# magicat777/Audio-Analyzer-OMEGA

Hardware: AMD Instinct MI355X
Metric: audio frames/sec (multi-res FFT + LUFS + TruePeak) at 1/2/4/8 MI355X (higher is better)
Workload: dtype f32; 1 GPU; cfg2: 256 stereo frames x 16384 samples per GPU; MRFFT 16k/8k/4k/1k + combine(512) + K-weighted LUFS + 4x true peak + meter aggregates; channel_frames_per_gpu=512, frame_samples=16384, target_bins=512, parallelism=frames sharded over 1 GPU(s)

## Files before the change

audio-analyzer-omega_amd/csrc/regfft.hpp:

```cpp
#pragma once
#include "fft.hpp"

namespace omega {

__device__ constexpr float kCos128[16] = {
    1.000000000e+00f, 9.987954562e-01f, 9.951847267e-01f, 9.891765100e-01f, 9.807852804e-01f,
    9.700312532e-01f, 9.569403357e-01f, 9.415440652e-01f, 9.238795325e-01f, 9.039892931e-01f,
    8.819212643e-01f, 8.577286100e-01f, 8.314696123e-01f, 8.032075315e-01f, 7.730104534e-01f,
    7.409511254e-01f};
__device__ constexpr float kSin128[16] = {
    0.000000000e+00f, 4.906767433e-02f, 9.801714033e-02f, 1.467304745e-01f, 1.950903220e-01f,
    2.429801799e-01f, 2.902846773e-01f, 3.368898534e-01f, 3.826834324e-01f, 4.275550934e-01f,
    4.713967368e-01f, 5.141027442e-01f, 5.555702330e-01f, 5.956993045e-01f, 6.343932842e-01f,
    6.715589548e-01f};

__device__ __forceinline__ void wave_lds_sync() {
  asm volatile("s_waitcnt lgkmcnt(0)" ::: "memory");
  __builtin_amdgcn_wave_barrier();
}

__device__ __forceinline__ float lane_xor1(float v) {
  return __int_as_float(__builtin_amdgcn_mov_dpp(__float_as_int(v), 0xB1, 0xF, 0xF, true));
}

__device__ __forceinline__ void lane_pair_fmac(float2 (&v)[16], float s) {
  asm volatile(
      "s_nop 1\n"
      "v_fmac_f32_dpp %0, %0, %32 quad_perm:[1,0,3,2] row_mask:0xf bank_mask:0xf\n"
      "v_fmac_f32_dpp %1, %1, %32 quad_perm:[1,0,3,2] row_mask:0xf bank_mask:0xf\n"
      "v_fmac_f32_dpp %2, %2, %32 quad_perm:[1,0,3,2] row_mask:0xf bank_mask:0xf\n"
      "v_fmac_f32_dpp %3, %3, %32 quad_perm:[1,0,3,2] row_mask:0xf bank_mask:0xf\n"
      "v_fmac_f32_dpp %4, %4, %32 quad_perm:[1,0,3,2] row_mask:0xf bank_mask:0xf\n"
      "v_fmac_f32_dpp %5, %5, %32 quad_perm:[1,0,3,2] row_mask:0xf bank_mask:0xf\n"
      "v_fmac_f32_dpp %6, %6, %32 quad_perm:[1,0,3,2] row_mask:0xf bank_mask:0xf\n"
      "v_fmac_f32_dpp %7, %7, %32 quad_perm:[1,0,3,2] row_mask:0xf bank_mask:0xf\n"
      "v_fmac_f32_dpp %8, %8, %32 quad_perm:[1,0,3,2] row_mask:0xf bank_mask:0xf\n"
      "v_fmac_f32_dpp %9, %9, %32 quad_perm:[1,0,3,2] row_mask:0xf bank_mask:0xf\n"
      "v_fmac_f32_dpp %10, %10, %32 quad_perm:[1,0,3,2] row_mask:0xf bank_mask:0xf\n"
      "v_fmac_f32_dpp %11, %11, %32 quad_perm:[1,0,3,2] row_mask:0xf bank_mask:0xf\n"
      "v_fmac_f32_dpp %12, %12, %32 quad_perm:[1,0,3,2] row_mask:0xf bank_mask:0xf\n"
      "v_fmac_f32_dpp %13, %13, %32 quad_perm:[1,0,3,2] row_mask:0xf bank_mask:0xf\n"
      "v_fmac_f32_dpp %14, %14, %32 quad_perm:[1,0,3,2] row_mask:0xf bank_mask:0xf\n"
      "v_fmac_f32_dpp %15, %15, %32 quad_perm:[1,0,3,2] row_mask:0xf bank_mask:0xf\n"
      "v_fmac_f32_dpp %16, %16, %32 quad_perm:[1,0,3,2] row_mask:0xf bank_mask:0xf\n"
      "v_fmac_f32_dpp %17, %17, %32 quad_perm:[1,0,3,2] row_mask:0xf bank_mask:0xf\n"
      "v_fmac_f32_dpp %18, %18, %32 quad_perm:[1,0,3,2] row_mask:0xf bank_mask:0xf\n"
      "v_fmac_f32_dpp %19, %19, %32 quad_perm:[1,0,3,2] row_mask:0xf bank_mask:0xf\n"
      "v_fmac_f32_dpp %20, %20, %32 quad_perm:[1,0,3,2] row_mask:0xf bank_mask:0xf\n"
      "v_fmac_f32_dpp %21, %21, %32 quad_perm:[1,0,3,2] row_mask:0xf bank_mask:0xf\n"
      "v_fmac_f32_dpp %22, %22, %32 quad_perm:[1,0,3,2] row_mask:0xf bank_mask:0xf\n"
      "v_fmac_f32_dpp %23, %23, %32 quad_perm:[1,0,3,2] row_mask:0xf bank_mask:0xf\n"
      "v_fmac_f32_dpp %24, %24, %32 quad_perm:[1,0,3,2] row_mask:0xf bank_mask:0xf\n"
      "v_fmac_f32_dpp %25, %25, %32 quad_perm:[1,0,3,2] row_mask:0xf bank_mask:0xf\n"
      "v_fmac_f32_dpp %26, %26, %32 quad_perm:[1,0,3,2] row_mask:0xf bank_mask:0xf\n"
      "v_fmac_f32_dpp %27, %27, %32 quad_perm:[1,0,3,2] row_mask:0xf bank_mask:0xf\n"
      "v_fmac_f32_dpp %28, %28, %32 quad_perm:[1,0,3,2] row_mask:0xf bank_mask:0xf\n"
      "v_fmac_f32_dpp %29, %29, %32 quad_perm:[1,0,3,2] row_mask:0xf bank_mask:0xf\n"
      "v_fmac_f32_dpp %30, %30, %32 quad_perm:[1,0,3,2] row_mask:0xf bank_mask:0xf\n"
      "v_fmac_f32_dpp %31, %31, %32 quad_perm:[1,0,3,2] row_mask:0xf bank_mask:0xf\n"
      : "+v"(v[0].x), "+v"(v[0].y),
        "+v"(v[1].x), "+v"(v[1].y),
        "+v"(v[2].x), "+v"(v[2].y),
        "+v"(v[3].x), "+v"(v[3].y),
        "+v"(v[4].x), "+v"(v[4].y),
        "+v"(v[5].x), "+v"(v[5].y),
        "+v"(v[6].x), "+v"(v[6].y),
        "+v"(v[7].x), "+v"(v[7].y),
        "+v"(v[8].x), "+v"(v[8].y),
        "+v"(v[9].x), "+v"(v[9].y),
        "+v"(v[10].x), "+v"(v[10].y),
        "+v"(v[11].x), "+v"(v[11].y),
        "+v"(v[12].x), "+v"(v[12].y),
        "+v"(v[13].x), "+v"(v[13].y),
        "+v"(v[14].x), "+v"(v[14].y),
        "+v"(v[15].x), "+v"(v[15].y)
      : "v"(s));
}

struct WinGen {
  float c0, c1, c2;
  float4 base;
  float4 step[8];
  __device__ __forceinline__ WinGen(const float4* __restrict__ g, int t) {
    const float4 c = g[0];
    c0 = c.x;
    c1 = c.y;
    c2 = c.z;
#pragma unroll
    for (int i = 0; i < 8; ++i) step[i] = g[1 + i];
    base = g[9 + t];
  }
  template <int Q, bool C2 = true>
  __device__ __forceinline__ float2 at() const {
    const float4 s4 = step[Q / 2];
    const float cs = (Q & 1) ? s4.z : s4.x, sn = (Q & 1) ? s4.w : s4.y;
    const float C0 = fmaf(base.x, cs, -base.y * sn), C1 = fmaf(base.z, cs, -base.w * sn);
    if constexpr (C2) return make_float2(fmaf(C0, fmaf(c2, C0, c1), c0), fmaf(C1, fmaf(c2, C1, c1), c0));
    else return make_float2(fmaf(C0, c1, c0), fmaf(C1, c1, c0));
  }
};

template <int K>
struct RegFFT {
  static_assert(K == 8192 || K == 4096, "register FFT plans: K = 4096, 8192");
  static constexpr int NTH = K / 16;
  static constexpr int L = K / 256;
  static constexpr int P1 = L == 32 ? 544 : 272;
  static constexpr int P2R = L == 32 ? 544 : 272;
  static constexpr int P2C = L == 32 ? 34 : 17;
  static_assert(P1 == P2R && 16 * P2R <= (K == 8192 ? 8712 : 4352), "exchange rows shared by both exchanges");
  static constexpr int kSlots = K == 8192 ? 8712 : 4352;
  static constexpr int kT2 = 15 * L;

  static __device__ __forceinline__ int a3(int n) {
    if constexpr (K == 8192) return n + (n >> 4) + ((n >> 12) << 3);
    else return n ^ ((n >> 4) & 15);
  }
  static __device__ __forceinline__ int s3(int t) {
    if constexpr (K == 8192) return t + (t >> 4);
    else return t ^ ((t >> 4) & 15);
  }
  static constexpr int o3(int r) { return K == 8192 ? 544 * r + 8 * (r >> 3) : 256 * r; }
  static __device__ __forceinline__ int s3m(int t) { return s3(NTH - t); }
  static __device__ __forceinline__ int out_index(int s, int m) {
    if constexpr (L == 32) return (s >> 5) + 16 * ((s >> 1) & 15) + 256 * (m + 16 * (s & 1));
    else return (s >> 4) + 16 * (s & 15) + 256 * m;
  }
  static __device__ __forceinline__ int s3o(int s) {
    if constexpr (L == 32) return (s >> 5) + 17 * ((s >> 1) & 15) + 4360 * (s & 1);
    else return ((s >> 4) ^ (s & 15)) + 16 * (s & 15);
  }
  static constexpr int o3o(int m) { return L == 32 ? 272 * m : 256 * m; }

  static __device__ __forceinline__ void twiddle(float2 (&v)[16], float2 w) {
    float2 wk = w;
    static_for<1, 16>([&](auto k) {
      v[k] = cmul(v[k], wk);
      if constexpr (k + 1 < 16) wk = cmul(wk, w);
    });
  }

  static __device__ __forceinline__ void dft16(float2 (&v)[16]) { dft16_fma(v); }

  static __device__ __forceinline__ void fill_t2(float2* t2, const float2* __restrict__ twK, int tid) {
    for (int i = tid; i < kT2; i += NTH) {
      const int k2 = i / L + 1, u = i % L;
      t2[i] = twK[(16 * u * k2) & (K - 1)];
    }
  }
  static __device__ __forceinline__ void twiddle_t2(float2 (&v)[16], const float2* t2u) {
    static_for<1, 16>([&](auto k2) { v[k2] = cmul(v[k2], t2u[(k2 - 1) * L]); });
  }

  template <bool SYNC = false, bool LT2 = false>
  static __device__ __forceinline__ void run(float2 (&v)[16], float2* buf, int t, float2 w1, float2 w2,
                                             const float2* t2 = nullptr) {
    run2<SYNC, LT2>(v, buf, t, t, w1, w2, t2);
  }
  template <bool SYNC = false, bool LT2 = false>
  static __device__ __forceinline__ void run2(float2 (&v)[16], float2* buf, int t1, int t, float2 w1, float2 w2,
                                              const float2* t2 = nullptr) {
    dft16(v);
    twiddle(v, w1);
    if constexpr (SYNC) __syncthreads();
    {
      float2* b = buf + t1;
      static_for<0, 16>([&](auto k1) { b[P1 * k1] = v[k1]; });
    }
    __syncthreads();
    {
      const int u = t % L, k1 = t / L;
      const float2* b = buf + P1 * k1 + u;
      static_for<0, 16>([&](auto r) { v[r] = b[L * r]; });
      dft16(v);
      if constexpr (LT2)
        twiddle_t2(v, t2 + u);
      else
        twiddle(v, w2);
      float2* bw = buf + P2R * k1 + u;
      static_for<0, 16>([&](auto k2) { bw[P2C * k2] = v[k2]; });
    }
    wave_lds_sync();
    if constexpr (L == 16) {
      const int k2 = t & 15, k1 = t >> 4;
      const float2* b = buf + P2R * k1 + P2C * k2;
      static_for<0, 16>([&](auto r) { v[r] = b[r]; });
      dft16(v);
    } else {
      const int q = t & 1, k2 = (t >> 1) & 15, k1 = t >> 5;
      const float2* b = buf + P2R * k1 + P2C * k2 + q;
      static_for<0, 16>([&](auto r) { v[r] = b[2 * r]; });
      dft16(v);
      static_for<0, 16>([&](auto m) {
        const float2 tw = twc<m + 16, 32>(v[m]);
        v[m] = make_float2(q ? tw.x : v[m].x, q ? tw.y : v[m].y);
      });
      lane_pair_fmac(v, q ? 1.f : -1.f);
    }
  }

  template <bool SYNC = false, bool LT2 = false>
  static __device__ __forceinline__ void run_low(float2 (&v)[16], float2* buf, int t, float2 w1, float2 w2,
                                                 const float2* t2 = nullptr) {
    static_assert(L == 32, "the two-band pass 3 is the K = 8192 plan");
    dft16(v);
    twiddle(v, w1);
    if constexpr (SYNC) __syncthreads();
    {
      float2* b = buf + t;
      static_for<0, 16>([&](auto k1) { b[P1 * k1] = v[k1]; });
    }
    __syncthreads();
    {
      const int u = t % L, k1 = t / L;
      const float2* b = buf + P1 * k1 + u;
      static_for<0, 16>([&](auto r) { v[r] = b[L * r]; });
      dft16(v);
      if constexpr (LT2)
        twiddle_t2(v, t2 + u);
      else
        twiddle(v, w2);
      float2* bw = buf + P2R * k1 + u;
      static_for<0, 16>([&](auto k2) { bw[P2C * k2] = v[k2]; });
    }
    wave_lds_sync();
    const int q = t & 1, k2 = (t >> 1) & 15, k1 = t >> 5;
    {
      const float2* b = buf + P2R * k1 + P2C * k2 + q;
      static_for<0, 16>([&](auto r) { v[r] = b[2 * r]; });
    }
    float2 f0 = v[0], f15 = v[0];
    static_for<1, 16>([&](auto r) {
      f0 = cadd(f0, v[r]);
      f15 = cadd(f15, twc<15 * r, 16>(v[r]));
    });
    const float2 g = twc<15, 32>(f15);
    const float2 send = q ? f0 : f15;
    const float2 recv = make_float2(lane_xor1(send.x), lane_xor1(send.y));
    const float2 out = q ? csub(recv, g) : cadd(f0, recv);
    __syncthreads();
    buf[s3o(t) + (q ? o3o(15) : 0)] = out;
    __syncthreads();
  }

  template <bool LT2 = false>
  static __device__ __forceinline__ void run_half(float2 (&v)[16], float* bf, int t, float2 w1, float2 w2,
                                                  const float2* t2 = nullptr) {
    static_assert(L == 16, "the half-buffer plan is K = 4096");
    dft16(v);
    twiddle(v, w1);
    const int u = t % L, k1 = t / L;
    {
      float* b = bf + t;
      static_for<0, 16>([&](auto j) { b[P1 * j] = v[j].x; });
    }
    __syncthreads();
    {
      const float* b = bf + P1 * k1 + u;
      static_for<0, 16>([&](auto r) { v[r].x = b[L * r]; });
    }
    __syncthreads();
    {
      float* b = bf + t;
      static_for<0, 16>([&](auto j) { b[P1 * j] = v[j].y; });
    }
    __syncthreads();
    {
      const float* b = bf + P1 * k1 + u;
      static_for<0, 16>([&](auto r) { v[r].y = b[L * r]; });
    }
    dft16(v);
    if constexpr (LT2)
      twiddle_t2(v, t2 + u);
    else
      twiddle(v, w2);
    {
      float* bw = bf + P2R * k1 + u;
      static_for<0, 16>([&](auto j) { bw[P2C * j] = v[j].x; });
    }
    wave_lds_sync();
    const int k2 = t & 15, k1b = t >> 4;
    const float* br = bf + P2R * k1b + P2C * k2;
    static_for<0, 16>([&](auto r) { v[r].x = br[r]; });
    {
      float* bw = bf + P2R * k1 + u;
      static_for<0, 16>([&](auto j) { bw[P2C * j] = v[j].y; });
    }
    wave_lds_sync();
    static_for<0, 16>([&](auto r) { v[r].y = br[r]; });
    dft16(v);
  }
  template <bool IM>
  static __device__ __forceinline__ void store_spectrum_half(const float2 (&v)[16], float* bf, int t) {
    float* b = bf + s3o(t);
    static_for<0, 16>([&](auto m) { b[o3o(m)] = IM ? v[m].y : v[m].x; });
  }

  static __device__ __forceinline__ void store_spectrum(const float2 (&v)[16], float2* buf, int t) {
    float2* b = buf + s3o(t);
    static_for<0, 16>([&](auto m) { b[o3o(m)] = v[m]; });
  }
};

}
```

audio-analyzer-omega_amd/csrc/rfkern.hip:

```cpp
#include <cstdlib>

#include "stamps.hpp"

namespace omega {
OMEGA_STAMPS_DECL
OMEGA_WGTRACE_DECL
OMEGA_MARKS_DECL
}

#include "kw.hpp"
#include "meter_query.hpp"
#include "regfft.hpp"
#include "spectral.hpp"

namespace omega {

template <int K>
constexpr size_t t2_offset() { return (RegFFT<K>::kSlots + 8) * sizeof(float2) + 64; }
template <int K>
constexpr size_t lds_bytes() { return t2_offset<K>() + RegFFT<K>::kT2 * sizeof(float2); }
template <int K>
__device__ __forceinline__ float2* t2_table(char* smem) { return reinterpret_cast<float2*>(smem + t2_offset<K>()); }

template <int NTH>
__device__ __forceinline__ int tp_column(int tid) {
  const int w = tid >> 6, l = tid & 63;
  if (l < 32) return 32 * w + l;
  const int a = 32 * w + (63 - l);
  return a == 0 ? NTH / 2 : NTH - a;
}

__device__ __forceinline__ void max3_abs16(float& acc, const float2 (&a)[16]) {
  asm(
      "v_max3_f32 %0, |%1|, |%2|, %0\n"
      "v_max3_f32 %0, |%3|, |%4|, %0\n"
      "v_max3_f32 %0, |%5|, |%6|, %0\n"
      "v_max3_f32 %0, |%7|, |%8|, %0\n"
      "v_max3_f32 %0, |%9|, |%10|, %0\n"
      "v_max3_f32 %0, |%11|, |%12|, %0\n"
      "v_max3_f32 %0, |%13|, |%14|, %0\n"
      "v_max3_f32 %0, |%15|, |%16|, %0\n"
      "v_max3_f32 %0, |%17|, |%18|, %0\n"
      "v_max3_f32 %0, |%19|, |%20|, %0\n"
      "v_max3_f32 %0, |%21|, |%22|, %0\n"
      "v_max3_f32 %0, |%23|, |%24|, %0\n"
      "v_max3_f32 %0, |%25|, |%26|, %0\n"
      "v_max3_f32 %0, |%27|, |%28|, %0\n"
      "v_max3_f32 %0, |%29|, |%30|, %0\n"
      "v_max3_f32 %0, |%31|, |%32|, %0\n"
      : "+v"(acc)
      : "v"(a[0].x), "v"(a[0].y),
        "v"(a[1].x), "v"(a[1].y),
        "v"(a[2].x), "v"(a[2].y),
        "v"(a[3].x), "v"(a[3].y),
        "v"(a[4].x), "v"(a[4].y),
        "v"(a[5].x), "v"(a[5].y),
        "v"(a[6].x), "v"(a[6].y),
        "v"(a[7].x), "v"(a[7].y),
        "v"(a[8].x), "v"(a[8].y),
        "v"(a[9].x), "v"(a[9].y),
        "v"(a[10].x), "v"(a[10].y),
        "v"(a[11].x), "v"(a[11].y),
        "v"(a[12].x), "v"(a[12].y),
        "v"(a[13].x), "v"(a[13].y),
        "v"(a[14].x), "v"(a[14].y),
        "v"(a[15].x), "v"(a[15].y));
}

template <int K>
__device__ __forceinline__ void truepeak_rf_body(const SpectralParams& p, int64_t cf, int tid, char* smem) {
  using FFT = RegFFT<K>;
  constexpr int NTH = FFT::NTH, M = 2 * K;
  const int t = tp_column<NTH>(tid);
  float2* buf = reinterpret_cast<float2*>(smem);
  float* red = reinterpret_cast<float*>(smem + (FFT::kSlots + 8) * sizeof(float2));
  const int64_t f = cf / p.C, c = cf % p.C;
  const float2* x2 = reinterpret_cast<const float2*>(p.x + f * p.frame_stride + c * p.chan_stride);
  const float2* __restrict__ twK = p.tw[ilog2(K)];
  const float2* __restrict__ twM = p.tw[ilog2(M)];
  float2 v[16];
  float mx = 0.f;
  OMEGA_STAMP(0);
  const float2 w1 = twK[t], w2 = twK[16 * (tid % FFT::L)];
  const float2 wm = twM[t];
  const float2 rho = p.rot[t];
  float2* t2 = t2_table<K>(smem);
  FFT::fill_t2(t2, twK, tid);
  asm volatile("" ::: "memory");
  static_for<0, 16>([&](auto r) {
    v[r] = x2[t + NTH * r];
    mx = fmaxf(mx, fmaxf(fabsf(v[r].x), fabsf(v[r].y)));
  });
  asm volatile("" : "+v"(mx));
  OMEGA_STAMP(1);
  FFT::template run2<false, true>(v, buf, t, tid, w1, w2, t2);
  OMEGA_STAMP(2);
  __syncthreads();
  FFT::store_spectrum(v, buf, tid);
  __syncthreads();
  OMEGA_STAMP(3);
  float xn = 0.f;
  {
    const float2* bo = buf + FFT::s3(t);
    const float2* bm = buf + FFT::s3m(t);
    static_for<0, 16>([&](auto r) {
      const float2 a = bo[FFT::o3(r)];
      float2 b = bm[FFT::o3(15 - r)];
      if constexpr (K == 8192 && r == 8) {
        if (t == 0) b = a;
      }
      float2 xk, xkk;
      untangle(a, b, twc<r, 32>(wm), xk, xkk);
      if constexpr (r == 0) {
        if (t == 0) {
          xn = a.x - a.y;
          xk = make_float2(a.x + a.y, 0.f);
        }
      }
      v[r] = xk;
    });
  }
  float2 y[16];
  static_for<0, 16>([&](auto r) { y[r] = v[r]; });
  const float2 hz = make_float2(wm.y, wm.x);
  float fmx = 0.f;
  const int lane = tid & 63;
  const int mir_addr = 4 * ((t == 0 || t == NTH / 2) ? lane : lane ^ 63);
  OMEGA_STAMP(4);
#pragma unroll 1
  for (int P = 1; P <= 3; ++P) {
    int tl = t, tidl = tid;
    float2 w1l = w1, w2l = w2, rhol = rho, hzl = hz;
    asm volatile("" : "+v"(tl), "+v"(tidl), "+v"(w1l.x), "+v"(w1l.y), "+v"(w2l.x), "+v"(w2l.y));
    asm volatile("" : "+v"(rhol.x), "+v"(rhol.y), "+v"(hzl.x), "+v"(hzl.y));
    static_for<0, 16>([&](auto r) {
      const float2 rk = cmul(rhol, make_float2(kCos128[r], kSin128[r]));
      y[r] = cmul(y[r], rk);
    });
    if (!((p.tp_phases >> P) & 1)) continue;
    OMEGA_STAMP(1 + 4 * P);
    const float cp = P == 1 ? 7.071067812e-01f : (P == 2 ? 0.f : -7.071067812e-01f);
    OMEGA_STAMP(2 + 4 * P);
    static_for<0, 16>([&](auto r) {
      const float2 m = y[15 - r];
      float2 yp = make_float2(__int_as_float(__builtin_amdgcn_ds_bpermute(mir_addr, __float_as_int(m.x))),
                              -__int_as_float(__builtin_amdgcn_ds_bpermute(mir_addr, __float_as_int(m.y))));
      if constexpr (r == 0) {
        if (tl == 0) yp = make_float2(xn * cp, 0.f);
      } else {
        if (tl == 0) yp = cconj(y[16 - r]);
      }
      const float2 g = twc<-r, 32>(hzl);
      const float2 S = cadd(y[r], yp), D = csub(y[r], yp);
      v[r] = make_float2(fmaf(g.x, D.x, fmaf(-g.y, D.y, S.x)), fmaf(-g.x, D.y, fmaf(-g.y, D.x, -S.y)));
    });
    OMEGA_STAMP(3 + 4 * P);
    FFT::template run2<true, true>(v, buf, tl, tidl, w1l, w2l, t2);
    max3_abs16(fmx, v);
#if defined(OMEGA_EXP_STALL)
    asm volatile("s_sleep %0" ::"i"(OMEGA_EXP_STALL));
#endif
#if defined(OMEGA_EXP_VALU)
    {
      float d0 = fmx, d1 = mx, d2 = fmx + 1.f, d3 = mx + 1.f;
      asm volatile(".rept %4\n v_fma_f32 %0, %0, %5, %6\n v_fma_f32 %1, %1, %5, %6\n"
                   " v_fma_f32 %2, %2, %5, %6\n v_fma_f32 %3, %3, %5, %6\n .endr"
                   : "+v"(d0), "+v"(d1), "+v"(d2), "+v"(d3)
                   : "i"(OMEGA_EXP_VALU), "v"(0.5f), "v"(0.25f));
    }
#endif
    OMEGA_STAMP(4 + 4 * P);
  }
  const float peak = block_max<NTH>(fmaxf(mx, fmx * (0.5f / K)), red, tid);
  if (tid == 0) {
    const float db = peak < 1e-10f ? -100.0f : 20.0f * log10f(peak);
    if (p.tp_done) {
      __hip_atomic_store(reinterpret_cast<unsigned*>(p.tp_out + cf), __float_as_uint(db), __ATOMIC_RELAXED,
                         __HIP_MEMORY_SCOPE_AGENT);
      asm volatile("s_waitcnt vmcnt(0)" ::: "memory");
      __hip_atomic_fetch_add(p.tp_done, 1u, __ATOMIC_RELAXED, __HIP_MEMORY_SCOPE_AGENT);
    } else {
      p.tp_out[cf] = db;
    }
    if (p.tp_copy) p.tp_copy[cf] = db;
  }
}

template <int K>
__global__ __launch_bounds__(K / 16, 4) void truepeak_rf_kernel(SpectralParams p) {
  extern __shared__ __attribute__((aligned(16))) char smem[];
  OMEGA_WG_BEGIN();
  truepeak_rf_body<K>(p, blockIdx.x, threadIdx.x, smem);
  OMEGA_WG_END(1);
}

template <int K>
__device__ __forceinline__ void mrfft_rf_body(const SpectralParams& p, int r, int64_t cf, int t, char* smem) {
  using FFT = RegFFT<K>;
  constexpr int NTH = FFT::NTH, M = 2 * K;
  float2* buf = reinterpret_cast<float2*>(smem);
  const int64_t f = cf / p.C, c = cf % p.C;
  const ResParam& rp = p.res[r];
  const float2* x2 = reinterpret_cast<const float2*>(p.x + f * p.frame_stride + c * p.chan_stride + rp.offset);
  const float2* __restrict__ twK = p.tw[ilog2(K)];
  const float2* __restrict__ twM = p.tw[ilog2(M)];
  float2 v[16];
  const float2 w1 = twK[t], w2b = twK[16 * (t % FFT::L)];
  const float2 wm = twM[t];
  float2* t2 = t2_table<K>(smem);
  FFT::fill_t2(t2, twK, t);
  asm volatile("" ::: "memory");
  const float2* w2 = reinterpret_cast<const float2*>(rp.win);
  static_for<0, 16>([&](auto q) {
    const float2 a = x2[t + NTH * q], w = w2[t + NTH * q];
    v[q] = make_float2(a.x * w.x, a.y * w.y);
  });
  const int e0 = rp.ent_begin + t;
  CombEnt ent{};
  if (p.comb_out && e0 < rp.ent_end) ent = p.ent[e0];
  bool low = false;
  if constexpr (K == 8192) low = !rp.mag_out && rp.low_band;
  if (low) {
    if constexpr (K == 8192) FFT::template run_low<false, true>(v, buf, t, w1, w2b, t2);
  } else {
    FFT::template run<false, true>(v, buf, t, w1, w2b, t2);
    __syncthreads();
    FFT::store_spectrum(v, buf, t);
    __syncthreads();
  }
  if (!rp.mag_out) {
    if (!p.comb_out) return;
    auto mag_at = [&](int j) -> float {
      const float2 a = buf[FFT::a3(j == K ? 0 : j)];
      if (j == 0) return fabsf(a.x + a.y);
      if (j == K) return fabsf(a.x - a.y);
      if (j == K / 2) return cabs(a);
      const float2 b = buf[FFT::a3(K - j)];
      float2 xk, xkk;
      untangle(a, b, twM[j], xk, xkk);
      return cabs(xk);
    };
    float* o = p.comb_out + cf * p.T;
    auto apply = [&](const CombEnt& en) {
      const int tt = en.tm & 0xFFFFFF, op = en.tm >> 24;
      if (op == 2) {
        o[tt] = 0.f;
        return;
      }
      const float val = fmaf(en.c1, mag_at(en.j + 1), en.c0 * mag_at(en.j));
      if (op == 0)
        o[tt] = val;
      else
        o[tt] += val;
    };
    if (e0 < rp.ent_end) apply(ent);
    for (int e = e0 + NTH; e < rp.ent_end; e += NTH) apply(p.ent[e]);
    return;
  }
  float mg[16];
  float mnyq = 0.f;
  {
    const float2* bo = buf + FFT::s3(t);
    const float2* bm = buf + FFT::s3m(t);
    static_for<0, 16>([&](auto q) {
      const float2 a = bo[FFT::o3(q)];
      float2 b = bm[FFT::o3(15 - q)];
      if constexpr (K == 8192 && q == 8) {
        if (t == 0) b = a;
      }
      float2 xk, xkk;
      untangle(a, b, twc<q, 32>(wm), xk, xkk);
      mg[q] = cabs(xk);
      if constexpr (q == 0) {
        if (t == 0) {
          mg[0] = fabsf(a.x + a.y);
          mnyq = fabsf(a.x - a.y);
        }
      }
    });
  }
  if (rp.mag_out) {
    float* o = rp.mag_out + cf * (K + 1);
    const float* __restrict__ wgt = rp.wgt;
    static_for<0, 16>([&](auto q) { o[t + NTH * q] = mg[q] * wgt[t + NTH * q]; });
    if (t == 0) o[K] = mnyq * wgt[K];
  }
  if (!p.comb_out) return;
  float* mag = reinterpret_cast<float*>(smem);
  __syncthreads();
  static_for<0, 16>([&](auto q) { mag[t + NTH * q] = mg[q]; });
  if (t == 0) mag[K] = mnyq;
  __syncthreads();
  float* o = p.comb_out + cf * p.T;
  auto apply = [&](const CombEnt& en) {
    const int tt = en.tm & 0xFFFFFF, op = en.tm >> 24;
    const float val = fmaf(en.c1, mag[en.j + 1], en.c0 * mag[en.j]);
    if (op == 0)
      o[tt] = val;
    else if (op == 1)
      o[tt] += val;
    else
      o[tt] = 0.f;
  };
  if (e0 < rp.ent_end) apply(ent);
  for (int e = e0 + NTH; e < rp.ent_end; e += NTH) apply(p.ent[e]);
}

template <int K>
__global__ __launch_bounds__(K / 16, 4) void mrfft_rf_kernel(SpectralParams p, int r) {
  extern __shared__ __attribute__((aligned(16))) char smem[];
  OMEGA_WG_BEGIN();
  mrfft_rf_body<K>(p, r, blockIdx.x, threadIdx.x, smem);
  OMEGA_WG_END(2);
}

OMEGA_STAMPS_GETTER(omega_debug_rf_stamps)
OMEGA_WGTRACE_GETTER(omega_debug_wgtrace)
OMEGA_MARKS_GETTER(omega_debug_marks_batch)

hipError_t launch_mrfft_rf(int n, const SpectralParams& p, int r, hipStream_t s) {
  const dim3 grid((unsigned)p.n_cf);
  if (n == 16384) {
    hipLaunchKernelGGL(mrfft_rf_kernel<8192>, grid, dim3(512), lds_bytes<8192>(), s, p, r);
  } else if (n == 8192) {
    hipLaunchKernelGGL(mrfft_rf_kernel<4096>, grid, dim3(256), lds_bytes<4096>(), s, p, r);
  } else {
    return hipErrorInvalidValue;
  }
  return hipGetLastError();
}

constexpr int kSpecRfThreads = 256;
#ifndef OMEGA_SPEC_WGS
#define OMEGA_SPEC_WGS 5
#endif
constexpr int kSpecRfWgs = OMEGA_SPEC_WGS;
constexpr int kSpecRfPeakWords = 12;
template <int K>
struct SpecRfLds {
  static constexpr size_t kT2Off = RegFFT<K>::kSlots * sizeof(float);
  static constexpr size_t kXform = kT2Off + RegFFT<K>::kT2 * sizeof(float2);
  static constexpr size_t kPartOff = ((K + 1) * sizeof(float) + 15) / 16 * 16;
  static constexpr size_t kClsOff = kPartOff + 240 * 5 * sizeof(float);
  static constexpr size_t kRedOff = kClsOff + 12 * 5 * sizeof(double);
  static constexpr size_t kFlagOff = (kRedOff + (RegFFT<K>::NTH / 64) * sizeof(float) + 15) / 16 * 16;
  static constexpr int kFlagWords = 2 * 64 * kSpecRfPeakWords / 4;
  static constexpr size_t kPost = kFlagOff + kFlagWords * sizeof(unsigned);
  static constexpr size_t kBytes = kXform > kPost ? kXform : kPost;
  static_assert((kBytes + 1279) / 1280 * 1280 * kSpecRfWgs <= 160 * 1024, "LDS of kSpecRfWgs workgroups per CU");
};


template <int K>
__device__ __forceinline__ void spectra_rf_body(const SpectraParams& p) {
  using FFT = RegFFT<K>;
  constexpr int NTH = FFT::NTH;
  static_assert(NTH == kSpecRfThreads, "one 256-thread workgroup per frame");
  extern __shared__ __attribute__((aligned(16))) char smem[];
  using Lds = SpecRfLds<K>;
  float* bf = reinterpret_cast<float*>(smem);
  float* magc = reinterpret_cast<float*>(smem);
  constexpr int kFlagWords = Lds::kFlagWords;
  float* part = reinterpret_cast<float*>(smem + Lds::kPartOff);
  double(*cls)[5] = reinterpret_cast<double(*)[5]>(smem + Lds::kClsOff);
  float* redf = reinterpret_cast<float*>(smem + Lds::kRedOff);
  unsigned* sflag = reinterpret_cast<unsigned*>(smem + Lds::kFlagOff);
  const int t = threadIdx.x;
  const int64_t fr = blockIdx.x;
  const float2* x2 = reinterpret_cast<const float2*>(p.x + fr * p.stride);
  float2 v[16];
  const float2* __restrict__ twK = p.tw[ilog2(K)];
  const float2 w1 = twK[t], w2b = twK[16 * (t % FFT::L)];
  const float2 wm = p.tw[ilog2(2 * K)][t];
  float2* t2 = reinterpret_cast<float2*>(smem + Lds::kT2Off);
  FFT::fill_t2(t2, twK, t);
  constexpr int kGrp = 20;
  int bs[2] = {0, 0}, be[2] = {0, 0};
  float bsc[2] = {1.f, 1.f};
  static_for<0, 2>([&](auto j) {
    const int i = t + NTH * j;
    if (p.bands_out && i < p.n_valid) {
      bs[j] = p.starts[i];
      be[j] = p.ends[i];
      if (p.scale) bsc[j] = p.scale[i];
    }
  });
  int cj0 = 0, cj1 = 0;
  if (p.chroma_out && t < 12 * kGrp) {
    cj0 = p.cgoff[t / kGrp];
    cj1 = p.cgoff[t / kGrp + 1];
  }
  const WinGen wg(p.wgen, t);
  asm volatile("" ::: "memory");
  OMEGA_STAMP_RT(30);
  OMEGA_STAMP(0);
  if (wg.c2 == 0.f) {
    static_for<0, 16>([&](auto r) {
      const float2 a = x2[t + NTH * r], w = wg.template at<r, false>();
      v[r] = make_float2(a.x * w.x, a.y * w.y);
    });
  } else {
    static_for<0, 16>([&](auto r) {
      const float2 a = x2[t + NTH * r], w = wg.template at<r>();
      v[r] = make_float2(a.x * w.x, a.y * w.y);
    });
  }
  OMEGA_STAMP(1);
  FFT::template run_half<true>(v, bf, t, w1, w2b, t2);
  OMEGA_STAMP(2);
  constexpr int kRecPre = 2, kRecReg = 8;
  float3 ra[kRecReg];
  const float3* __restrict__ crec = reinterpret_cast<const float3*>(p.crec);
  int cjf = cj0 + t % kGrp;
  static_for<0, kRecPre>([&](auto i) {
    const int j = cjf + kGrp * i;
    if (j < cj1) {
      ra[i] = crec[j];
    }
  });
  asm volatile("" ::: "memory");
  float ax[8], bx[8], ay[8], by[8];
  float hx = 0.f, hy = 0.f;
  {
    const float* bo = bf + FFT::s3(t);
    const float* bm = bf + FFT::s3m(t);
    __syncthreads();
    FFT::template store_spectrum_half<false>(v, bf, t);
    __syncthreads();
    static_for<0, 8>([&](auto q) {
      ax[q] = bo[FFT::o3(q)];
      bx[q] = bm[FFT::o3(15 - q)];
    });
    if (t == 0) hx = bo[FFT::o3(8)];
    __syncthreads();
    FFT::template store_spectrum_half<true>(v, bf, t);
    __syncthreads();
    static_for<0, 8>([&](auto q) {
      ay[q] = bo[FFT::o3(q)];
      by[q] = bm[FFT::o3(15 - q)];
    });
    if (t == 0) hy = bo[FFT::o3(8)];
  }
  OMEGA_STAMP(3);
  float mg[8], mgm[8];
  float mx = 0.f, mhalf = 0.f;
  {
    static_for<0, 8>([&](auto q) {
      const float2 a = make_float2(ax[q], ay[q]);
      const float2 b = make_float2(bx[q], by[q]);
      float2 xk, xkk;
      untangle(a, b, twc<q, 32>(wm), xk, xkk);
      mg[q] = cabs(xk);
      mgm[q] = cabs(xkk);
      if constexpr (q == 0) {
        if (t == 0) {
          mg[0] = fabsf(a.x + a.y);
          mgm[0] = fabsf(a.x - a.y);
        }
      }
      mx = fmaxf(mx, fmaxf(mg[q], mgm[q]));
    });
    if (t == 0) {
      mhalf = cabs(make_float2(hx, hy));
      mx = fmaxf(mx, mhalf);
    }
  }
  mx = wave_max(mx);
  __syncthreads();
  static_for<0, 8>([&](auto q) {
    magc[t + NTH * q] = mg[q];
    magc[K - t - NTH * q] = mgm[q];
  });
  if (t == 0) magc[K / 2] = mhalf;
  if ((t & 63) == 0) redf[t >> 6] = mx;
  for (int i = t; i < kFlagWords; i += NTH) sflag[i] = 0u;
  OMEGA_STAMP(4);
  __syncthreads();
  float thr = redf[0];
#pragma unroll
  for (int w = 1; w < NTH / 64; ++w) thr = fmaxf(thr, redf[w]);
  thr *= 0.1f;
  if (p.chroma_out && t < 12 * kGrp) {
    static_for<0, kRecReg>([&](auto i) {
      const int j = cjf + kGrp * i;
      if (i >= kRecPre && j < cj1) {
        ra[i] = crec[j];
      }
    });
  }
  OMEGA_STAMP(5);
  if (p.mag_out) {
    float* o = p.mag_out + fr * (K + 1);
    static_for<0, 8>([&](auto q) {
      o[t + NTH * q] = mg[q];
      o[K - t - NTH * q] = mgm[q];
    });
    if (t == 0) o[K / 2] = mhalf;
  }
  if (p.bands_out) {
    float* o = p.bands_out + fr * p.n_out;
    auto band = [&](int i, int s, int e, float scale) {
      float val = 0.f;
      if (i < p.n_valid && s < K + 1 && e <= K + 1) {
        float m0 = magc[s], m1 = m0, m2 = m0, m3 = m0;
        int k = s + 1;
        for (; k + 3 < e; k += 4) {
          m0 = fmaxf(m0, magc[k]);
          m1 = fmaxf(m1, magc[k + 1]);
          m2 = fmaxf(m2, magc[k + 2]);
          m3 = fmaxf(m3, magc[k + 3]);
        }
        for (; k < e; ++k) m0 = fmaxf(m0, magc[k]);
        val = fmaxf(fmaxf(m0, m1), fmaxf(m2, m3)) * scale;
      }
      o[i] = val;
    };
    static_for<0, 2>([&](auto j) {
      const int i = t + NTH * j;
      if (i < p.n_out) {
        band(i, bs[j], be[j], bsc[j]);
      }
    });
    for (int i = t + 2 * NTH; i < p.n_out; i += NTH) {
      float val = 0.f;
      if (i < p.n_valid) {
        const int s = p.starts[i], e = p.ends[i];
        if (s < K + 1 && e <= K + 1) {
          float m0 = magc[s], m1 = m0, m2 = m0, m3 = m0;
          int k = s + 1;
          for (; k + 3 < e; k += 4) {
            m0 = fmaxf(m0, magc[k]);
            m1 = fmaxf(m1, magc[k + 1]);
            m2 = fmaxf(m2, magc[k + 2]);
            m3 = fmaxf(m3, magc[k + 3]);
          }
          for (; k < e; ++k) m0 = fmaxf(m0, magc[k]);
          val = fmaxf(fmaxf(m0, m1), fmaxf(m2, m3)) * (p.scale ? p.scale[i] : 1.f);
        }
      }
      o[i] = val;
    }
  }
  OMEGA_STAMP(6);
  if (!p.chroma_out) return;
  {
    const int lane = t & 63;
    static_for<0, kSpecRfPeakWords / (NTH / 64)>([&](auto q) {
      const int k = t + NTH * q;
      const float val = mg[q];
      float lo = wave_shift1<true>(val), hi = wave_shift1<false>(val);
      if (lane == 0) lo = k >= 1 ? magc[k - 1] : 0.f;
      if (lane == 63) hi = magc[k + 1];
      if (k >= 1 && k <= K - 1 && val > lo && val > hi && val > thr) {
        static_for<2, 6>([&](auto h) {
          const int kh = k * h;
          if (kh >= p.c_lo && kh < p.c_hi) atomicOr(&sflag[kh >> 2], 1u << (8 * (kh & 3) + h));
        });
      }
    });
  }
  __syncthreads();
  OMEGA_STAMP(7);
  auto suppressed = [&](int k) {
    const unsigned f = (sflag[k >> 2] >> (8 * (k & 3))) & 0xFFu;
    float m = magc[k];
    m = (f & 32u) ? m * (1.0f / 5) : m;
    m = (f & 16u) ? m * (1.0f / 4) : m;
    m = (f & 8u) ? m * (1.0f / 3) : m;
    m = (f & 4u) ? m * (1.0f / 2) : m;
    return m;
  };
  OMEGA_STAMP(8);
  if (t < 12 * kGrp) {
    float acc[5] = {0.f, 0.f, 0.f, 0.f, 0.f};
    const int j1 = cj1;
    auto acc_rec = [&](const float3 r) {
      const float ed = suppressed(__float_as_int(r.z));
      const float a = r.x, g = r.y, gi = __builtin_amdgcn_rcpf(g);
      const float ag = a * g, agi = a * gi;
      acc[0] = fmaf(ed, agi * (gi * 3.3546262790251185e-4f), acc[0]);
      acc[1] = fmaf(ed, agi * 1.3533528323661270e-1f, acc[1]);
      acc[2] = fmaf(ed, a, acc[2]);
      acc[3] = fmaf(ed, ag * 1.3533528323661270e-1f, acc[3]);
      acc[4] = fmaf(ed, ag * (g * 3.3546262790251185e-4f), acc[4]);
    };
    static_for<0, kRecReg>([&](auto i) {
      if (cjf + kGrp * i < j1) acc_rec(ra[i]);
    });
    for (int j = cjf + kGrp * kRecReg; j < j1; j += kGrp) acc_rec(crec[j]);
#pragma unroll
    for (int o = 0; o < 5; ++o) part[t * 5 + o] = acc[o];
  }
  OMEGA_STAMP(9);
  __syncthreads();
  OMEGA_STAMP(10);
  if (t < 60 * 4) {
    const int pr = t >> 2, k = t & 3, g = pr / 5, o = pr % 5;
    const float* pp = part + (g * kGrp + 5 * k) * 5 + o;
    double sgo = (double)pp[0];
#pragma unroll
    for (int r = 1; r < 5; ++r) sgo += (double)pp[5 * r];
    sgo += __shfl_xor(sgo, 1, 64);
    sgo += __shfl_xor(sgo, 2, 64);
    if (k == 0) cls[(g + o + 10) % 12][o] = sgo;
  }
  __syncthreads();
  if (t < 64) {
    const int c = t % 12;
    const double ch = cls[c][0] + cls[c][1] + cls[c][2] + cls[c][3] + cls[c][4];
    const int cm = (c + 11) % 12, cp = (c + 1) % 12;
    const double chm = cls[cm][0] + cls[cm][1] + cls[cm][2] + cls[cm][3] + cls[cm][4];
    const double chp = cls[cp][0] + cls[cp][1] + cls[cp][2] + cls[cp][3] + cls[cp][4];
    const double sm = 0.25 * chm + 0.5 * ch + 0.25 * chp;
    double tot = t < 12 ? sm : 0.0;
    tot += __shfl_xor(tot, 8, 64);
    tot += __shfl_xor(tot, 4, 64);
    tot += __shfl_xor(tot, 2, 64);
    tot += __shfl_xor(tot, 1, 64);
    if (t < 12) p.chroma_out[fr * 12 + c] = tot > 0 ? sm / tot : sm;
  }
  OMEGA_STAMP(11);
  OMEGA_STAMP_RT(31);
}

template <int K>
__global__ __launch_bounds__(kSpecRfThreads, kSpecRfWgs) void spectra_rf_kernel(SpectraParams p) {
  OMEGA_WG_BEGIN();
  spectra_rf_body<K>(p);
  OMEGA_WG_END(20);
}

hipError_t launch_spectra_rf(int m, const SpectraParams& p, hipStream_t s) {
  if (m != 8192 || (p.chroma_out && p.c_hi > 2 * 64 * kSpecRfPeakWords)) return hipErrorInvalidValue;
  hipLaunchKernelGGL(spectra_rf_kernel<4096>, dim3((unsigned)p.n), dim3(kSpecRfThreads), SpecRfLds<4096>::kBytes,
                     s, p);
  return hipGetLastError();
}

hipError_t launch_truepeak_rf(int W, const SpectralParams& p, hipStream_t s, int extra_lds) {
  const dim3 grid((unsigned)p.n_cf);
  if (W == 16384) {
    hipLaunchKernelGGL(truepeak_rf_kernel<8192>, grid, dim3(512), lds_bytes<8192>() + extra_lds, s, p);
  } else if (W == 8192) {
    hipLaunchKernelGGL(truepeak_rf_kernel<4096>, grid, dim3(256), lds_bytes<4096>(), s, p);
  } else {
    return hipErrorInvalidValue;
  }
  return hipGetLastError();
}

constexpr int kBatchThreads = 512;

template <int K>
__device__ __forceinline__ void batch_multi(const SpectralParams& p, int r, int64_t wg, int tid, float2* smem) {
  constexpr int G = threads_for<K>();
  constexpr int FPW = kBatchThreads / G;
  static_assert(FPW * K * sizeof(float2) <= lds_bytes<8192>(), "LDS of one batch workgroup");
  const int grp = tid / G;
  const int64_t cf = wg * FPW + grp;
  const bool valid = cf < p.n_cf;
  mrfft_frame<K, G>(p, r, valid ? cf : p.n_cf - 1, valid, tid % G, smem + grp * K);
}

__device__ __forceinline__ void batch_kw_role(const KWeightParams& kp, int64_t cf, int tid, char* smem) {
  constexpr int kP = 2 * kPwl * 16;
  auto* pwl = reinterpret_cast<float4(*)[kPwl]>(smem);
  float* fbuf = reinterpret_cast<float*>(smem + kP);
  float* sh = reinterpret_cast<float*>(smem + kP + 65536);
  float* edge = sh + 36;
  double* red = reinterpret_cast<double*>(smem + kP + 65536 + 224);
  static_assert(kP + 65536 + 224 + 64 <= lds_bytes<8192>(), "K-weighting role LDS");
  kweight_body<16384, kBatchThreads, true, true>(kp, cf, tid, pwl, fbuf, sh, edge, red);
  kw_count_in(kp, tid);
}

__device__ __forceinline__ void batch_meter_role(const MeterPrepParams& mp, int q, int nq, int tid) {
  const int64_t n_out = mp.n_frames * mp.C, step = (int64_t)nq * (kBatchThreads / 64);
  const int64_t o0 = (int64_t)q * (kBatchThreads / 64) + (tid >> 6);
  const int lane = tid & 63;
  OMEGA_MARK(q, 0);
  if (tid == 0) poll_count(mp.start_ctr, mp.start_target, mp.poll_limit, mp.err_word + 1);
  __syncthreads();
  OMEGA_MARK(q, 1);
  for (int64_t o = o0; o < n_out; o += step) meter_query_wave(mp, o / mp.C, (int)(o % mp.C), lane, true, false);
  const float th0 = o0 < n_out ? tp_hist_part(mp, o0 / mp.C, (int)(o0 % mp.C), lane) : -INFINITY;
  OMEGA_MARK(q, 2);
  if (tid == 0) poll_count(mp.join_ctr, mp.join_target, mp.poll_limit, mp.err_word + 1);
  __syncthreads();
  OMEGA_MARK(q, 3);
  const int64_t n_roll = (int64_t)mp.C * mp.HT, roll_step = (int64_t)nq * kBatchThreads;
  int64_t e = (int64_t)q * kBatchThreads + tid;
  float rv = 0.f;
  const int64_t rdst = e < n_roll ? tp_roll_load(mp, e, rv) : -1;
  for (int64_t o = o0; o < n_out; o += step) {
    const int64_t f = o / mp.C;
    const int c = (int)(o % mp.C);
    tp_finish(mp, f, c, lane, o == o0 ? th0 : tp_hist_part(mp, f, c, lane));
  }
  if (rdst >= 0) mp.hist_t_out[rdst] = rv;
  for (e += roll_step; e < n_roll; e += roll_step) {
    const int64_t d = tp_roll_load(mp, e, rv);
    if (d >= 0) mp.hist_t_out[d] = rv;
  }
  if (mp.seg_ctr) {
    asm volatile("s_waitcnt vmcnt(0)" ::: "memory");
    __syncthreads();
    if (tid == 0) __hip_atomic_fetch_add(mp.seg_ctr, 1u, __ATOMIC_RELAXED, __HIP_MEMORY_SCOPE_AGENT);
  }
  OMEGA_MARK(q, 4);
}

__device__ __forceinline__ void batch_body(const SpectralParams& sp, const KWeightParams& kp, const BatchPlan& bp,
                                           const MeterPrepParams& mq, char* smem) {
  const int tid = threadIdx.x;
  const int b = blockIdx.x;
  OMEGA_WG_BEGIN();
  if (bp.tail_ctr && b == (int)gridDim.x - 1 && tid == 0)
    __hip_atomic_fetch_add(bp.tail_ctr, 1u, __ATOMIC_RELAXED, __HIP_MEMORY_SCOPE_SYSTEM);
  if (b >= bp.q_begin && b < bp.q_begin + bp.q_n) {
    batch_meter_role(mq, b - bp.q_begin, bp.q_n, tid);
    OMEGA_WG_END(4);
    return;
  }

  const int len0 = bp.seg_begin[1], len1 = bp.seg_begin[2] - bp.seg_begin[1];
  const int sg = (b >= bp.seg_start[0] && b < bp.seg_start[0] + len0) ? 0
                 : (b >= bp.seg_start[1] && b < bp.seg_start[1] + len1) ? 1 : -1;
  if (sg >= 0) {
    const int j = b - bp.seg_start[sg], nr = bp.n_roles[sg];
    int role;
    int64_t cf;
    if (nr == 2 && bp.pat == 1) {
      const int g = j >> 3, per = g & 7, rb = (0x5A >> per) & 1;
      role = bp.roles[sg][rb];
      const int idx = 4 * (g >> 3) + __popc((rb ? 0x5A : 0xA5) & ((1 << per) - 1));
      cf = (int64_t)idx * 8 + (j & 7);
    } else {
      role = bp.roles[sg][(j >> 3) % nr];
      cf = (int64_t)(j / (8 * nr)) * 8 + (j & 7);
    }
    if (cf >= sp.n_cf) return;
    if (role == 0) {
      batch_kw_role(kp, cf, tid, smem);
    } else if (role == 1) {
      truepeak_rf_body<8192>(sp, cf, tid, smem);
    } else {
      mrfft_rf_body<8192>(sp, bp.mr_res, cf, tid, smem);
    }
    OMEGA_WG_END(role);
    return;
  }
  const MultiPlan& mp = bp.multi;
  const int w = b - bp.multi_start -
                (b >= bp.q_begin + bp.q_n && bp.q_begin < bp.multi_start + bp.multi_n ? bp.q_n : 0);
  if (w < 0 || w >= bp.multi_n) return;
  int s = 0;
  while (s + 1 < mp.n_seg && w >= mp.wg_begin[s + 1]) ++s;
  const int r = mp.res[s];
  const int64_t wg = w - mp.wg_begin[s];
  float2* buf = reinterpret_cast<float2*>(smem);
  switch (sp.res[r].n) {
    case 512: batch_multi<256>(sp, r, wg, tid, buf); break;
    case 1024: batch_multi<512>(sp, r, wg, tid, buf); break;
    case 2048: batch_multi<1024>(sp, r, wg, tid, buf); break;
    case 4096: batch_multi<2048>(sp, r, wg, tid, buf); break;
    case 8192: batch_multi<4096>(sp, r, wg, tid, buf); break;
    default: break;
  }
  OMEGA_WG_END(3 + sp.res[r].n);
}

__global__ __launch_bounds__(kBatchThreads, 4) void batch_kernel(SpectralParams sp, KWeightParams kp, BatchPlan bp,
                                                                 MeterPrepParams mq) {
  extern __shared__ __attribute__((aligned(16))) char smem[];
  batch_body(sp, kp, bp, mq, smem);
}

hipError_t launch_batch(const SpectralParams& sp, const KWeightParams& kp, const BatchPlan& bp, const MeterPrepParams& mq,
                        int grid, hipStream_t s) {
  hipLaunchKernelGGL(batch_kernel, dim3((unsigned)grid), dim3(kBatchThreads), lds_bytes<8192>(), s, sp, kp, bp, mq);
  return hipGetLastError();
}

}
```

Baseline: 8.408 million channel-frames/s.

## Fold true-peak phase rotation into constant twiddles and unroll phase loop

```diff
diff --git a/audio-analyzer-omega_amd/csrc/regfft.hpp b/audio-analyzer-omega_amd/csrc/regfft.hpp
--- a/audio-analyzer-omega_amd/csrc/regfft.hpp
+++ b/audio-analyzer-omega_amd/csrc/regfft.hpp
@@ -3,16 +3,31 @@
 
 namespace omega {
 
-__device__ constexpr float kCos128[16] = {
-    1.000000000e+00f, 9.987954562e-01f, 9.951847267e-01f, 9.891765100e-01f, 9.807852804e-01f,
-    9.700312532e-01f, 9.569403357e-01f, 9.415440652e-01f, 9.238795325e-01f, 9.039892931e-01f,
-    8.819212643e-01f, 8.577286100e-01f, 8.314696123e-01f, 8.032075315e-01f, 7.730104534e-01f,
-    7.409511254e-01f};
-__device__ constexpr float kSin128[16] = {
-    0.000000000e+00f, 4.906767433e-02f, 9.801714033e-02f, 1.467304745e-01f, 1.950903220e-01f,
-    2.429801799e-01f, 2.902846773e-01f, 3.368898534e-01f, 3.826834324e-01f, 4.275550934e-01f,
-    4.713967368e-01f, 5.141027442e-01f, 5.555702330e-01f, 5.956993045e-01f, 6.343932842e-01f,
-    6.715589548e-01f};
+constexpr float cos128(int j) {
+  constexpr float q[33] = {
+      1.000000000e+00f, 9.987954497e-01f, 9.951847196e-01f, 9.891765118e-01f, 9.807852507e-01f,
+      9.700312614e-01f, 9.569403529e-01f, 9.415440559e-01f, 9.238795042e-01f, 9.039893150e-01f,
+      8.819212914e-01f, 8.577286005e-01f, 8.314695954e-01f, 8.032075167e-01f, 7.730104327e-01f,
+      7.409511209e-01f, 7.071067691e-01f, 6.715589762e-01f, 6.343932748e-01f, 5.956993103e-01f,
+      5.555702448e-01f, 5.141027570e-01f, 4.713967443e-01f, 4.275550842e-01f, 3.826834261e-01f,
+      3.368898630e-01f, 2.902846634e-01f, 2.429801822e-01f, 1.950903237e-01f, 1.467304677e-01f,
+      9.801714122e-02f, 4.906767607e-02f, 0.000000000e+00f};
+  j = ((j % 128) + 128) % 128;
+  if (j > 64) j = 128 - j;
+  return j <= 32 ? q[j] : -q[64 - j];
+}
+constexpr float sin128(int j) { return cos128(j - 32); }
+
+template <int J>
+__device__ __forceinline__ float2 rot128(float2 z) {
+  constexpr int j = ((J % 128) + 128) % 128;
+  if constexpr (j % 4 == 0) {
+    return twc<-(j / 4), 32>(z);
+  } else {
+    constexpr float c = cos128(j), s = sin128(j);
+    return make_float2(fmaf(z.x, c, -(z.y * s)), fmaf(z.x, s, z.y * c));
+  }
+}
 
 __device__ __forceinline__ void wave_lds_sync() {
   asm volatile("s_waitcnt lgkmcnt(0)" ::: "memory");
@@ -139,6 +154,13 @@
       if constexpr (k + 1 < 16) wk = cmul(wk, w);
     });
   }
+  static __device__ __forceinline__ void twiddle(float2 (&v)[16], float2 w, float2 w0) {
+    float2 wk = w0;
+    static_for<0, 16>([&](auto k) {
+      v[k] = cmul(v[k], wk);
+      if constexpr (k + 1 < 16) wk = cmul(wk, w);
+    });
+  }
 
   static __device__ __forceinline__ void dft16(float2 (&v)[16]) { dft16_fma(v); }
 
@@ -157,11 +179,14 @@
                                              const float2* t2 = nullptr) {
     run2<SYNC, LT2>(v, buf, t, t, w1, w2, t2);
   }
-  template <bool SYNC = false, bool LT2 = false>
+  template <bool SYNC = false, bool LT2 = false, bool W0 = false>
   static __device__ __forceinline__ void run2(float2 (&v)[16], float2* buf, int t1, int t, float2 w1, float2 w2,
-                                              const float2* t2 = nullptr) {
-    dft16(v);
-    twiddle(v, w1);
+                                              const float2* t2 = nullptr, float2 w0 = float2{1.f, 0.f}) {
+    dft16(v);
+    if constexpr (W0)
+      twiddle(v, w1, w0);
+    else
+      twiddle(v, w1);
     if constexpr (SYNC) __syncthreads();
     {
       float2* b = buf + t1;
diff --git a/audio-analyzer-omega_amd/csrc/rfkern.hip b/audio-analyzer-omega_amd/csrc/rfkern.hip
--- a/audio-analyzer-omega_amd/csrc/rfkern.hip
+++ b/audio-analyzer-omega_amd/csrc/rfkern.hip
@@ -127,35 +127,50 @@
   const int lane = tid & 63;
   const int mir_addr = 4 * ((t == 0 || t == NTH / 2) ? lane : lane ^ 63);
   OMEGA_STAMP(4);
-#pragma unroll 1
-  for (int P = 1; P <= 3; ++P) {
+  static_for<1, 4>([&](auto Pc) {
+    constexpr int P = Pc;
+    if (!((p.tp_phases >> P) & 1)) return;
     int tl = t, tidl = tid;
     float2 w1l = w1, w2l = w2, rhol = rho, hzl = hz;
     asm volatile("" : "+v"(tl), "+v"(tidl), "+v"(w1l.x), "+v"(w1l.y), "+v"(w2l.x), "+v"(w2l.y));
     asm volatile("" : "+v"(rhol.x), "+v"(rhol.y), "+v"(hzl.x), "+v"(hzl.y));
-    static_for<0, 16>([&](auto r) {
-      const float2 rk = cmul(rhol, make_float2(kCos128[r], kSin128[r]));
-      y[r] = cmul(y[r], rk);
-    });
-    if (!((p.tp_phases >> P) & 1)) continue;
     OMEGA_STAMP(1 + 4 * P);
-    const float cp = P == 1 ? 7.071067812e-01f : (P == 2 ? 0.f : -7.071067812e-01f);
+    float2 rp = rhol;
+    static_for<1, P>([&](auto) { rp = cmul(rp, rhol); });
+    constexpr float cp = P == 1 ? 7.071067812e-01f : (P == 2 ? 0.f : -7.071067812e-01f);
+    constexpr float nqx = P == 2 ? 0.f : 7.071067812e-01f * (P == 1 ? cp : -cp);
+    constexpr float nqy = P == 2 ? 0.f : -7.071067812e-01f * cp;
+    constexpr float h = 7.071067812e-01f;
     OMEGA_STAMP(2 + 4 * P);
     static_for<0, 16>([&](auto r) {
-      const float2 m = y[15 - r];
-      float2 yp = make_float2(__int_as_float(__builtin_amdgcn_ds_bpermute(mir_addr, __float_as_int(m.x))),
-                              -__int_as_float(__builtin_amdgcn_ds_bpermute(mir_addr, __float_as_int(m.y))));
+      const float2 ms = y[15 - r];
+      float2 m = make_float2(__int_as_float(__builtin_amdgcn_ds_bpermute(mir_addr, __float_as_int(ms.x))),
+                             __int_as_float(__builtin_amdgcn_ds_bpermute(mir_addr, __float_as_int(ms.y))));
       if constexpr (r == 0) {
-        if (tl == 0) yp = make_float2(xn * cp, 0.f);
+        if (tl == 0) m = make_float2(xn * nqx, xn * nqy);
       } else {
-        if (tl == 0) yp = cconj(y[16 - r]);
-      }
-      const float2 g = twc<-r, 32>(hzl);
-      const float2 S = cadd(y[r], yp), D = csub(y[r], yp);
-      v[r] = make_float2(fmaf(g.x, D.x, fmaf(-g.y, D.y, S.x)), fmaf(-g.x, D.y, fmaf(-g.y, D.x, -S.y)));
+        if (tl == 0) m = y[16 - r];
+      }
+      float2 S, D;
+      if constexpr (P == 2) {
+        S = make_float2(y[r].x - m.y, y[r].y - m.x);
+        D = make_float2(y[r].x + m.y, y[r].y + m.x);
+      } else {
+        const float d = m.x - m.y, s = m.x + m.y;
+        if constexpr (P == 1) {
+          S = make_float2(fmaf(h, d, y[r].x), fmaf(-h, s, y[r].y));
+          D = make_float2(fmaf(-h, d, y[r].x), fmaf(h, s, y[r].y));
+        } else {
+          S = make_float2(fmaf(-h, s, y[r].x), fmaf(-h, d, y[r].y));
+          D = make_float2(fmaf(h, s, y[r].x), fmaf(h, d, y[r].y));
+        }
+      }
+      const float2 G = rot128<r * (4 + P)>(hzl);
+      const float2 cS = rot128<r * P>(S);
+      v[r] = make_float2(fmaf(G.x, D.x, fmaf(-G.y, D.y, cS.x)), fmaf(-G.x, D.y, fmaf(-G.y, D.x, -cS.y)));
     });
     OMEGA_STAMP(3 + 4 * P);
-    FFT::template run2<true, true>(v, buf, tl, tidl, w1l, w2l, t2);
+    FFT::template run2<true, true, true>(v, buf, tl, tidl, w1l, w2l, t2, cconj(rp));
     max3_abs16(fmx, v);
 #if defined(OMEGA_EXP_STALL)
     asm volatile("s_sleep %0" ::"i"(OMEGA_EXP_STALL));
@@ -170,7 +185,7 @@
     }
 #endif
     OMEGA_STAMP(4 + 4 * P);
-  }
+  });
   const float peak = block_max<NTH>(fmaxf(mx, fmx * (0.5f / K)), red, tid);
   if (tid == 0) {
     const float db = peak < 1e-10f ? -100.0f : 20.0f * log10f(peak);
```

Result: no change. 8.408 million channel-frames/s (-0.0%).

## Fold per-lane phase rotation into FFT first-stage twiddle for true-peak phases

Applied to the files above, without the earlier changes.

```diff
diff --git a/audio-analyzer-omega_amd/csrc/regfft.hpp b/audio-analyzer-omega_amd/csrc/regfft.hpp
--- a/audio-analyzer-omega_amd/csrc/regfft.hpp
+++ b/audio-analyzer-omega_amd/csrc/regfft.hpp
@@ -13,6 +13,17 @@
     2.429801799e-01f, 2.902846773e-01f, 3.368898534e-01f, 3.826834324e-01f, 4.275550934e-01f,
     4.713967368e-01f, 5.141027442e-01f, 5.555702330e-01f, 5.956993045e-01f, 6.343932842e-01f,
     6.715589548e-01f};
+
+__device__ constexpr float kCos128h[16] = {
+    9.996988187e-01f, 9.972904567e-01f, 9.924795346e-01f, 9.852776424e-01f, 9.757021300e-01f,
+    9.637760658e-01f, 9.495281806e-01f, 9.329927988e-01f, 9.142097557e-01f, 8.932243012e-01f,
+    8.700869911e-01f, 8.448535652e-01f, 8.175848132e-01f, 7.883464276e-01f, 7.572088465e-01f,
+    7.242470830e-01f};
+__device__ constexpr float kSin128h[16] = {
+    2.454122852e-02f, 7.356456360e-02f, 1.224106752e-01f, 1.709618888e-01f, 2.191012402e-01f,
+    2.667127575e-01f, 3.136817404e-01f, 3.598950365e-01f, 4.052413140e-01f, 4.496113297e-01f,
+    4.928981922e-01f, 5.349976199e-01f, 5.758081914e-01f, 6.152315906e-01f, 6.531728430e-01f,
+    6.895405447e-01f};
 
 __device__ __forceinline__ void wave_lds_sync() {
   asm volatile("s_waitcnt lgkmcnt(0)" ::: "memory");
@@ -140,6 +151,14 @@
     });
   }
 
+  static __device__ __forceinline__ void twiddle0(float2 (&v)[16], float2 w, float2 w0) {
+    float2 wk = w0;
+    static_for<0, 16>([&](auto k) {
+      v[k] = cmul(v[k], wk);
+      if constexpr (k + 1 < 16) wk = cmul(wk, w);
+    });
+  }
+
   static __device__ __forceinline__ void dft16(float2 (&v)[16]) { dft16_fma(v); }
 
   static __device__ __forceinline__ void fill_t2(float2* t2, const float2* __restrict__ twK, int tid) {
@@ -157,11 +176,14 @@
                                              const float2* t2 = nullptr) {
     run2<SYNC, LT2>(v, buf, t, t, w1, w2, t2);
   }
-  template <bool SYNC = false, bool LT2 = false>
+  template <bool SYNC = false, bool LT2 = false, bool PRE = false>
   static __device__ __forceinline__ void run2(float2 (&v)[16], float2* buf, int t1, int t, float2 w1, float2 w2,
-                                              const float2* t2 = nullptr) {
-    dft16(v);
-    twiddle(v, w1);
+                                              const float2* t2 = nullptr, float2 w0 = make_float2(1.f, 0.f)) {
+    dft16(v);
+    if constexpr (PRE)
+      twiddle0(v, w1, w0);
+    else
+      twiddle(v, w1);
     if constexpr (SYNC) __syncthreads();
     {
       float2* b = buf + t1;
diff --git a/audio-analyzer-omega_amd/csrc/rfkern.hip b/audio-analyzer-omega_amd/csrc/rfkern.hip
--- a/audio-analyzer-omega_amd/csrc/rfkern.hip
+++ b/audio-analyzer-omega_amd/csrc/rfkern.hip
@@ -67,6 +67,31 @@
         "v"(a[15].x), "v"(a[15].y));
 }
 
+template <bool COL0>
+__device__ __forceinline__ void tp_pack(const float2 (&y)[16], float2 (&v)[16], int mir_addr, float2 hz, bool col0,
+                                        float xn, int P) {
+  const float2 nq = P == 1 ? make_float2(7.068938138e-01f, 1.735326911e-02f)
+                           : (P == 2 ? make_float2(0.f, 0.f) : make_float2(-7.051908447e-01f, -5.201800178e-02f));
+  const float2 e0 = P == 1 ? make_float2(kCos128[1], kSin128[1])
+                           : (P == 2 ? make_float2(kCos128[2], kSin128[2]) : make_float2(kCos128[3], kSin128[3]));
+  static_for<0, 16>([&](auto r) {
+    const float2 m = y[15 - r];
+    float2 yp = make_float2(__int_as_float(__builtin_amdgcn_ds_bpermute(mir_addr, __float_as_int(m.x))),
+                            -__int_as_float(__builtin_amdgcn_ds_bpermute(mir_addr, __float_as_int(m.y))));
+    if constexpr (COL0) {
+      if constexpr (r == 0) {
+        if (col0) yp = make_float2(xn * nq.x, xn * nq.y);
+      } else {
+        const float2 a = y[16 - r];
+        if (col0) yp = make_float2(fmaf(a.x, e0.x, a.y * e0.y), fmaf(a.x, e0.y, -a.y * e0.x));
+      }
+    }
+    const float2 g = twc<-r, 32>(hz);
+    const float2 S = cadd(y[r], yp), D = csub(y[r], yp);
+    v[r] = make_float2(fmaf(g.x, D.x, fmaf(-g.y, D.y, S.x)), fmaf(-g.x, D.y, fmaf(-g.y, D.x, -S.y)));
+  });
+}
+
 template <int K>
 __device__ __forceinline__ void truepeak_rf_body(const SpectralParams& p, int64_t cf, int tid, char* smem) {
   using FFT = RegFFT<K>;
@@ -126,36 +151,27 @@
   float fmx = 0.f;
   const int lane = tid & 63;
   const int mir_addr = 4 * ((t == 0 || t == NTH / 2) ? lane : lane ^ 63);
+  const float2 kap = cmul(rho, make_float2(9.996988187e-01f, -2.454122852e-02f));
+  float2 kq = make_float2(1.f, 0.f);
+  const bool wave0 = __builtin_amdgcn_readfirstlane(tid) < 64;
   OMEGA_STAMP(4);
 #pragma unroll 1
   for (int P = 1; P <= 3; ++P) {
     int tl = t, tidl = tid;
-    float2 w1l = w1, w2l = w2, rhol = rho, hzl = hz;
+    float2 w1l = w1, w2l = w2, kapl = kap, hzl = hz;
     asm volatile("" : "+v"(tl), "+v"(tidl), "+v"(w1l.x), "+v"(w1l.y), "+v"(w2l.x), "+v"(w2l.y));
-    asm volatile("" : "+v"(rhol.x), "+v"(rhol.y), "+v"(hzl.x), "+v"(hzl.y));
-    static_for<0, 16>([&](auto r) {
-      const float2 rk = cmul(rhol, make_float2(kCos128[r], kSin128[r]));
-      y[r] = cmul(y[r], rk);
-    });
+    asm volatile("" : "+v"(kapl.x), "+v"(kapl.y), "+v"(hzl.x), "+v"(hzl.y));
+    static_for<0, 16>([&](auto r) { y[r] = cmul(y[r], make_float2(kCos128h[r], kSin128h[r])); });
+    kq = cmul(kq, kapl);
     if (!((p.tp_phases >> P) & 1)) continue;
     OMEGA_STAMP(1 + 4 * P);
-    const float cp = P == 1 ? 7.071067812e-01f : (P == 2 ? 0.f : -7.071067812e-01f);
     OMEGA_STAMP(2 + 4 * P);
-    static_for<0, 16>([&](auto r) {
-      const float2 m = y[15 - r];
-      float2 yp = make_float2(__int_as_float(__builtin_amdgcn_ds_bpermute(mir_addr, __float_as_int(m.x))),
-                              -__int_as_float(__builtin_amdgcn_ds_bpermute(mir_addr, __float_as_int(m.y))));
-      if constexpr (r == 0) {
-        if (tl == 0) yp = make_float2(xn * cp, 0.f);
-      } else {
-        if (tl == 0) yp = cconj(y[16 - r]);
-      }
-      const float2 g = twc<-r, 32>(hzl);
-      const float2 S = cadd(y[r], yp), D = csub(y[r], yp);
-      v[r] = make_float2(fmaf(g.x, D.x, fmaf(-g.y, D.y, S.x)), fmaf(-g.x, D.y, fmaf(-g.y, D.x, -S.y)));
-    });
+    if (wave0)
+      tp_pack<true>(y, v, mir_addr, hzl, tl == 0, xn, P);
+    else
+      tp_pack<false>(y, v, mir_addr, hzl, false, xn, P);
     OMEGA_STAMP(3 + 4 * P);
-    FFT::template run2<true, true>(v, buf, tl, tidl, w1l, w2l, t2);
+    FFT::template run2<true, true, true>(v, buf, tl, tidl, w1l, w2l, t2, cconj(kq));
     max3_abs16(fmx, v);
 #if defined(OMEGA_EXP_STALL)
     asm volatile("s_sleep %0" ::"i"(OMEGA_EXP_STALL));
```

New measurement: 8.411 million channel-frames/s before, 8.444 million channel-frames/s after, median of 6. Within noise of the previous version (+0.4%).
